# ibrahimhroob/SPS

Measured on AMD Instinct MI355X. Metric: scans/sec @100k pts, 0.1 m voxel, higher is better.
Workload: dtype f32; 1 GPU; BASELINE config 2: single ~100k-pt LiDAR-like scan + variant-B submap, 0.1 m voxel, CustomMinkUNet14 fp32, 1 scan per step per GPU (4 distinct scans cycled); scan_points=100824, rows=153557, streams_per_gpu=8, compact_arenas=True

## Files before the change

### sps_amd/csrc/conv_kernels.inc.h

```cpp

typedef float floatx4 __attribute__((ext_vector_type(4)));

struct ConvArgs {
  const float *in;
  float *out;
  const float *Wu;
  const float *scale;
  const float *shift;
  const float *res;
  const int *nbr;
  const uint32_t *tmask;
  const int *n_out;
  const int *abort_flag;
  int out_rows;
  int64_t ldn;
  int ldi, ldo, ldr;
  int K, cin, cout, NT, upk;
  int relu, S;
  float inv_upk;
  float in_const;
  uint32_t in_bytes, wu_bytes, nbr_bytes;
  int tile_cap;
  int trace_on;
  const float *in2;
// ... 829 lines not shown
#pragma unroll
          for (int i = 0; i < 4; ++i)
            rv[i] = __uint_as_float(__builtin_amdgcn_raw_buffer_load_b32(
                rsR, child[i] >= 0 ? ((uint32_t)child[i] * (uint32_t)a.ldr + (uint32_t)col) * 4u : 0xFFFFFFFFu, 0, 0));
        }
#pragma unroll
        for (int i = 0; i < 4; ++i) {
          if (child[i] < 0) continue;
          float y = acc[nt][i] * esc[nt] + esh[nt];
          y += rv[i];
          if (a.relu) y = fmaxf(y, 0.f);
          a.out[(size_t)child[i] * a.ldo + col] = y;
        }
      }
    }
  }
}

__global__ __launch_bounds__(256) void k_conv0_fused(const int *__restrict__ n_out, LevelView L,
                                                      const float *__restrict__ W, const float *__restrict__ scale,
                                                      const float *__restrict__ shift, float in_const,
                                                      float *__restrict__ out, int ldo, int relu, TileOrderArgs to, int g0) {
  __shared__ float w_s[128 * 8];
  const int gto = (int)gridDim.x - g0;
  if ((int)blockIdx.x < gto) {
    const int which = (int)blockIdx.x;
    if (which < NLV - TILE_ORDER_FIRST_LEVEL)
      tile_order_body(to, which);
    else
      px_order_body(to, which - (NLV - TILE_ORDER_FIRST_LEVEL));
    return;
  }
  const int bid = (int)blockIdx.x - gto;
  if (n_out[ABORT]) return;
  for (int i = threadIdx.x; i < 128 * 8; i += blockDim.x) w_s[i] = i < 125 * 8 ? W[i] : 0.f;
  __syncthreads();
  const int n = *n_out;
  const int ntiles = (n + 15) >> 4;
  const int lane = threadIdx.x & 63, wave = __builtin_amdgcn_readfirstlane((int)(threadIdx.x >> 6));
  const int r = lane & 15, q = lane >> 4;
  const float esc = r < 8 ? scale[r] : 0.f, esh = r < 8 ? shift[r] : 0.f;
  const __amdgpu_buffer_rsrc_t rsM = __builtin_amdgcn_make_buffer_rsrc((void *)L.bmask, 0, (int)0xFFFFFFFEu, 0x00020000);
  for (int tile = bid * 4 + wave; tile < ntiles; tile += g0 * 4) {
    const int row0 = tile * 16;
    const int u = row0 + r;
    uint32_t bm[4] = {0u, 0u, 0u, 0u};
#if defined(SPS_ABLATE_C0FETCH)
    bm[0] = bm[1] = 0x0F0F0F0Fu;
    if (false) {
      const int blk = L.vblock[u];
#else
    if (u < n) {
      const int blk = L.vblock[u];
#endif
      const int bit = L.vbit[u];
      const int px = bit & 3, py = (bit >> 2) & 3, pz = bit >> 4;
      const int lx = px < 2 ? -1 : 0, ly = py < 2 ? -1 : 0, lz = pz < 2 ? -1 : 0;
      const int ysel = q & 1, zsel = q >> 1;
      const int *adj = L.badj + (size_t)blk * 81 + 27 + (lz + zsel + 1) * 9 + (ly + ysel + 1) * 3 + (lx + 1);
      const int nb0 = adj[0], nb1 = adj[1];
      const u32x2 M0 = __builtin_amdgcn_raw_buffer_load_b64(rsM, nb0 >= 0 ? (uint32_t)nb0 * 8u : 0xFFFFFFFFu, 0, 0);
      const u32x2 M1 = __builtin_amdgcn_raw_buffer_load_b64(rsM, nb1 >= 0 ? (uint32_t)nb1 * 8u : 0xFFFFFFFFu, 0, 0);
      const uint32_t m0lo = M0.x, m0hi = M0.y, m1lo = M1.x, m1hi = M1.y;
      const int ysplit = 4 * (ly + 1), zsplit = 4 * (lz + 1);
      const int ty0 = ysel ? ysplit : py - 2, ty1 = ysel ? py + 2 : ysplit - 1;
      const int tz0 = zsel ? zsplit : pz - 2, tz1 = zsel ? pz + 2 : zsplit - 1;
      const int xs = px - 2 - 4 * lx;
#pragma unroll 1
      for (int iz = 0; iz < 4; ++iz) {
        const int tz = tz0 + iz;
        const bool hiw = (tz & 2) != 0;
        const uint32_t w0 = hiw ? m0hi : m0lo, w1 = hiw ? m1hi : m1lo;
        uint32_t plane = 0u;
#pragma unroll
        for (int iy = 0; iy < 4; ++iy) {
          const int ty = ty0 + iy;
          const bool on = tz <= tz1 && ty <= ty1;
          const int sh = ((tz & 1) << 4) | ((ty & 3) << 2);
          const uint32_t n0 = (w0 >> sh) & 0xFu, n1 = (w1 >> sh) & 0xFu;
          const uint32_t pres = on ? (((n0 | (n1 << 4)) >> xs) & 0x1Fu) : 0u;
          plane |= pres << (5 * iy);
        }
        const int k0 = 5 * ((ty0 - py + 2) + 5 * (tz - pz + 2));
        const unsigned long long wide = (unsigned long long)plane << (k0 & 31);
        const int wi = (k0 >> 5) & 3;
        bm[0] |= wi == 0 ? (uint32_t)wide : 0u;
        bm[1] |= wi == 1 ? (uint32_t)wide : (wi == 0 ? (uint32_t)(wide >> 32) : 0u);
        bm[2] |= wi == 2 ? (uint32_t)wide : (wi == 1 ? (uint32_t)(wide >> 32) : 0u);
// ... 173 lines not shown
```

### sps_amd/csrc/grid_kernels.inc.h

```cpp

typedef unsigned int u32x2 __attribute__((ext_vector_type(2)));
constexpr int SCAN_BLOCK = 1024;

struct BHash {
  uint64_t *keys;
  unsigned long long *mask;
  int *first;
  int *rank;
  uint32_t *occ;
  uint32_t hmask;
  uint32_t hshift;
};

constexpr uint32_t BH_X = 0x9E3779B1u, BH_Y = 0x85EBCA77u, BH_Z = 0xC2B2AE3Du, BH_T = 0x27D4EB2Fu;
__device__ inline uint32_t bhash32(uint64_t key) {
  return (uint32_t)(key & 0x3FFFF) * BH_X + (uint32_t)((key >> 18) & 0x3FFFF) * BH_Y + (uint32_t)((key >> 36) & 0x3FFFF) * BH_Z +
         (uint32_t)(key >> 54) * BH_T;
}

__device__ inline int bhash_insert(const BHash &h, uint64_t key) {
  uint32_t s = bhash32(key) >> h.hshift;
  while (true) {
    unsigned long long prev = atomicCAS(reinterpret_cast<unsigned long long *>(&h.keys[s]),
                                        (unsigned long long)KEY_EMPTY, (unsigned long long)key);
// ... 106 lines not shown
  uint64_t *bkey[NLV];
  unsigned long long *bmask[NLV];
  int *bbase[NLV];
  uint4 *bmb[NLV];
  int *bparent[NLV];
  int *bchild[NLV];
  int *badj[NLV];
  int *vblock[NLV];
  unsigned char *vbit[NLV];
  int *counts;
  unsigned long long *agg;
  int agg_stride;
  uint32_t gen;
  const int *n_dev;
  int capl[NLV], bcapl[NLV];
  int *err;
};

constexpr int ABORT = 15;

__device__ inline int block_reduce_sum(int v, int *lds) {
  const int lane = threadIdx.x & 63, wave = threadIdx.x >> 6;
  for (int o = 32; o > 0; o >>= 1) v += __shfl_down(v, o, 64);
  if (lane == 0) lds[wave] = v;
  __syncthreads();
  int tot = 0;
  const int nw = blockDim.x >> 6;
  for (int i = 0; i < nw; ++i) tot += lds[i];
  __syncthreads();
  return tot;
}

constexpr int TICKET = 16, TOCC = 24, N_COUNTERS = 32;

__device__ inline unsigned long long agg_pack(uint32_t gen, int t0, int t1) {
  return ((unsigned long long)gen << 32) | ((unsigned long long)(uint32_t)t1 << 13) | (unsigned long long)(uint32_t)t0;
}
constexpr int SCAN_SPIN_MAX = 1 << 22;
__device__ inline int2 scan_lookback(const unsigned long long *agg, int id, uint32_t gen, int *lds, int *err) {
  if constexpr (SPS_ABLATE_FE & 2) return make_int2(0, 0);
  int p0 = 0, p1 = 0;
  for (int i = threadIdx.x; i < id; i += SCAN_BLOCK) {
    unsigned long long v = __hip_atomic_load(agg + i, __ATOMIC_RELAXED, __HIP_MEMORY_SCOPE_AGENT);
    for (int spin = 0; (uint32_t)(v >> 32) != gen; ++spin) {
      if (spin == SCAN_SPIN_MAX) {
        atomicOr(err, 16);
        v = 0ull;
        break;
      }
      __builtin_amdgcn_s_sleep(1);
      v = __hip_atomic_load(agg + i, __ATOMIC_RELAXED, __HIP_MEMORY_SCOPE_AGENT);
    }
    p0 += (int)(v & 0x1FFFull);
    p1 += (int)((v >> 13) & 0x7FFFFull);
  }
  const int b0 = block_reduce_sum(p0, lds);
  const int b1 = block_reduce_sum(p1, lds);
  return make_int2(b0, b1);
}
__device__ inline int2 block_exclusive_scan2(int v0, int v1, int2 *wave_off, int2 &tot) {
  const int lane = threadIdx.x & 63, wave = threadIdx.x >> 6;
  int i0 = v0, i1 = v1;
  for (int o = 1; o < 64; o <<= 1) {
    const int t0 = __shfl_up(i0, o, 64), t1 = __shfl_up(i1, o, 64);
    if (lane >= o) {
      i0 += t0;
// ... 152 lines not shown
            for (int i = 0; i < 2; ++i)
              if (m & (0x0000000000330033ull << (2 * i + 8 * jj + 32 * kk)))
                pm |= 1ull << ((2 * oz + kk) * 16 + (2 * oy + jj) * 4 + (2 * ox + i));
      } else {
        const uint32_t px = (bx >> (l - 2)) & 3, py = (by >> (l - 2)) & 3, pz = (bz >> (l - 2)) & 3;
        pm = 1ull << ((pz << 4) | (py << 2) | px);
      }
    }
    const int r = k.wg_rank0 + j;
    int sl = 0;
    if constexpr (!(SPS_ABLATE_FE & 4))
      sl = wave_run_insert(a.h[l], pkey, ok, (uint32_t)pm, (uint32_t)(pm >> 32), r);
    if (ok) a.sslot[l][r] = sl;
  }
#if defined(SPS_FE_TRACE)
  __syncthreads();
  FE_STAMP(0, 6);
#endif
}

constexpr int RANK_ITEMS = 1;
__global__ __launch_bounds__(SCAN_BLOCK) void k_rank_blocks_rows(PyramidArgs a, int gsb, int n0, int *__restrict__ inv) {
  __shared__ int lds[SCAN_BLOCK / 64];
  __shared__ int2 wave_off[SCAN_BLOCK / 64];
  __shared__ int sh_id;
  if ((int)blockIdx.x < 4 * gsb) {
    const int nblk = a.counts[8];
    if (((int)blockIdx.x % gsb) * (SCAN_BLOCK * RANK_ITEMS) >= nblk) return;
    Ranked k;
    rank_pass<RANK_ITEMS>(a, 1 + (int)blockIdx.x / gsb, nblk, k, lds, wave_off, &sh_id);
    FE_STAMP(1, 4);
    return;
  }
  if (a.counts[ABORT]) return;
  FE_STAMP(1, 0);
  const int n = a.n_dev ? min(n0, *a.n_dev) : n0;
  const int p = ((int)blockIdx.x - 4 * gsb) * SCAN_BLOCK + (int)threadIdx.x;
  if (p >= n) return;
  const int s = a.sslot[0][p];
  int row = -1;
  if (s >= 0) {
    const BHash &h = a.h[0];
    const int r = h.rank[s];
    const int bit = a.sbit0[p];
    row = a.bbase[0][r] + __popcll(h.mask[s] & ((1ull << bit) - 1ull));
    a.vblock[0][row] = r;
    a.vbit[0][row] = (unsigned char)bit;
  }
  inv[p] = row;
  FE_STAMP(1, 6);
}

__device__ inline void link_levels(const PyramidArgs &a, int l, int bx, int nbx) {
  const int n = a.counts[8 + l];
  for (int r = bx * 256 + (int)threadIdx.x; r < n; r += nbx * 256) {
    const uint64_t key = a.bkey[l][r];
    const uint32_t bx = (uint32_t)(key & 0x3FFFF), by = (uint32_t)((key >> 18) & 0x3FFFF),
                   bz = (uint32_t)((key >> 36) & 0x3FFFF);
    const uint64_t bt = key & (0x3FFull << 54);
    const uint64_t pkey = bt | ((uint64_t)(bz >> 1) << 36) | ((uint64_t)(by >> 1) << 18) | (uint64_t)(bx >> 1);
    const int ps = bhash_find(a.h[l + 1], pkey);
    const int pr = a.h[l + 1].rank[ps];
    a.bparent[l][r] = pr;
    a.bchild[l + 1][(size_t)pr * 8 + ((bx & 1) | ((by & 1) << 1) | ((bz & 1) << 2))] = r;
    if (l == 0) {
      const unsigned long long m = a.bmask[0][r];
      int sj[NLV], brj[NLV], basej[NLV];
      unsigned long long pmj[NLV];
#pragma unroll
      for (int j = 1; j < NLV; ++j) sj[j] = a.sslot[j][r];
#pragma unroll
      for (int j = 1; j < NLV; ++j) {
        brj[j] = a.h[j].rank[sj[j]];
        pmj[j] = a.h[j].mask[sj[j]];
      }
#pragma unroll
      for (int j = 1; j < NLV; ++j) basej[j] = a.bbase[j][brj[j]];
#pragma unroll
      for (int j = 1; j < NLV; ++j) {
        const int br = brj[j];
        const unsigned long long pmask = pmj[j];
        const int base = basej[j];
        if (j == 1) {
          const uint32_t ox = bx & 1, oy = by & 1, oz = bz & 1;
#pragma unroll
          for (int k = 0; k < 2; ++k)
#pragma unroll
            for (int jj = 0; jj < 2; ++jj)
#pragma unroll
              for (int i = 0; i < 2; ++i)
                if (m & (0x0000000000330033ull << (2 * i + 8 * jj + 32 * k))) {
                  const int bit = (int)((2 * oz + k) * 16 + (2 * oy + jj) * 4 + (2 * ox + i));
                  const int row = base + __popcll(pmask & ((1ull << bit) - 1ull));
                  a.vblock[1][row] = br;
                  a.vbit[1][row] = (unsigned char)bit;
                }
        } else {
          const uint32_t px = (bx >> (j - 2)) & 3, py = (by >> (j - 2)) & 3, pz = (bz >> (j - 2)) & 3;
          const int bit = (int)((pz << 4) | (py << 2) | px);
          const int row = base + __popcll(pmask & ((1ull << bit) - 1ull));
          a.vblock[j][row] = br;
          a.vbit[j][row] = (unsigned char)bit;
        }
      }
    }
  }
}

constexpr int LINK_PER = 3;
#if defined(SPS_FE_TRACE)
__device__ unsigned long long g_link_trace[2 * 16384];
struct LinkStamp {
  __device__ LinkStamp() { if (threadIdx.x == 0 && blockIdx.x < 16384) g_link_trace[2 * blockIdx.x] = wall_clock64(); }
  __device__ ~LinkStamp() { if (threadIdx.x == 0 && blockIdx.x < 16384) g_link_trace[2 * blockIdx.x + 1] = wall_clock64(); }
};
#endif
__global__ __launch_bounds__(256) void k_link_adj(PyramidArgs a, int gb, int c1, int c2, int c3, int c4, int c5) {
  if (a.counts[ABORT]) return;
#if defined(SPS_FE_TRACE)
  LinkStamp stamp;
#endif
  if ((int)blockIdx.x < 4 * gb) {
    link_levels(a, (int)blockIdx.x / gb, (int)blockIdx.x % gb, gb);
    return;
  }
  const int bx = (int)blockIdx.x - 4 * gb;
  const int idx = bx < c1 ? 0 : bx < c2 ? 1 : bx < c3 ? 2 : bx < c4 ? 3 : 4;
  const int level = NLV - 1 - idx;
  const int lo = idx == 0 ? 0 : idx == 1 ? c1 : idx == 2 ? c2 : idx == 3 ? c3 : c4;
  const int hi = idx == 0 ? c1 : idx == 1 ? c2 : idx == 2 ? c3 : idx == 3 ? c4 : c5;
  const int total = a.counts[8 + level] * 27;
  const int lim = 1 << (16 - level);
  const BHash h = a.h[level];
  const uint32_t tocc = reinterpret_cast<const uint32_t *>(a.counts)[TOCC];
  const uint64_t *__restrict__ bkey = a.bkey[level];
  int *__restrict__ badj = a.badj[level];
  const __amdgpu_buffer_rsrc_t rsOcc = __builtin_amdgcn_make_buffer_rsrc((void *)h.occ, 0, (int)0xFFFFFFFEu, 0x00020000);
  const __amdgpu_buffer_rsrc_t rsKeys = __builtin_amdgcn_make_buffer_rsrc((void *)h.keys, 0, (int)0xFFFFFFFEu, 0x00020000);
  const __amdgpu_buffer_rsrc_t rsRank = __builtin_amdgcn_make_buffer_rsrc((void *)h.rank, 0, (int)0xFFFFFFFEu, 0x00020000);
  for (int i = (bx - lo) * 256 + (int)threadIdx.x; i < total; i += (hi - lo) * 256) {
    const int r = i / 27, g = i - r * 27;
    const int dy = g % 3 - 1, dz = (g / 3) % 3 - 1, dt = g / 9 - 1;
    const uint64_t key = bkey[r];
    const int kx = (int)(key & 0x3FFFF), ky = (int)((key >> 18) & 0x3FFFF) + dy, kz = (int)((key >> 36) & 0x3FFFF) + dz,
              tt = (int)((key >> 54) & 0x1F) + dt;
    const bool gok = ky >= 0 && ky < lim && kz >= 0 && kz < lim && tt >= 0 && tt < 32 && ((tocc >> tt) & 1u);
    const uint64_t gkey = key + ((uint64_t)(int64_t)dy << 18) + ((uint64_t)(int64_t)dz << 36) + ((uint64_t)(int64_t)dt << 54);
    const uint32_t ghash = bhash32(key) + (uint32_t)dy * BH_Y + (uint32_t)dz * BH_Z + (uint32_t)dt * BH_T;
    uint64_t nk[LINK_PER];
    uint32_t sl[LINK_PER];
    int res[LINK_PER];
    bool probe[LINK_PER];
#pragma unroll
    for (int j = 0; j < LINK_PER; ++j) {
      const int dx = j - 1;
      const bool self = dx == 0 && g == 13;
      res[j] = self ? r : -1;
      probe[j] = !(SPS_ABLATE_FE & 8) && gok && !self && kx + dx >= 0 && kx + dx < lim;
      nk[j] = gkey + (uint64_t)(int64_t)dx;
      sl[j] = (ghash + (uint32_t)dx * BH_X) >> h.hshift;
    }
    uint32_t ow[LINK_PER];
#pragma unroll
    for (int j = 0; j < LINK_PER; ++j) ow[j] = __builtin_amdgcn_raw_buffer_load_b32(rsOcc, probe[j] ? (sl[j] >> 5) * 4u : 0xFFFFFFFFu, 0, 0);
    uint64_t k1[LINK_PER];
#pragma unroll
    for (int j = 0; j < LINK_PER; ++j) {
      probe[j] = probe[j] && ((ow[j] >> (sl[j] & 31)) & 1u);
      const u32x2 kv = __builtin_amdgcn_raw_buffer_load_b64(rsKeys, probe[j] ? sl[j] * 8u : 0xFFFFFFFFu, 0, 0);
      k1[j] = ((uint64_t)kv.y << 32) | kv.x;
    }
    bool hit[LINK_PER];
    int rk[LINK_PER];
#pragma unroll
    for (int j = 0; j < LINK_PER; ++j) {
      hit[j] = probe[j] && k1[j] == nk[j];
      rk[j] = (int)__builtin_amdgcn_raw_buffer_load_b32(rsRank, hit[j] ? sl[j] * 4u : 0xFFFFFFFFu, 0, 0);
    }
#pragma unroll
    for (int j = 0; j < LINK_PER; ++j) {
      if (hit[j]) {
        res[j] = rk[j];
      } else if (probe[j]) {
        const int s2 = bhash_find_from(h, nk[j], (sl[j] + 1) & h.hmask);
        if (s2 >= 0) res[j] = h.rank[s2];
      }
    }
    int *__restrict__ o = badj + (size_t)r * 81 + g * 3;
    if constexpr (SPS_ABLATE_FE & 16) {
      if (g == 13) o[1] = res[1];
    } else {
#pragma unroll
      for (int j = 0; j < LINK_PER; ++j) o[j] = res[j];
    }
  }
}

__device__ inline void bhash_cleanup(const PyramidArgs &a, int l, int bx, int nbx) {
  const int n = a.counts[8 + l];
  const BHash h = a.h[l];
  if (a.counts[ABORT]) {
    const uint32_t slots = h.hmask + 1u;
    for (uint32_t s = (uint32_t)bx * 256u + threadIdx.x; s < slots; s += (uint32_t)nbx * 256u) {
      h.keys[s] = KEY_EMPTY;
      h.mask[s] = 0ull;
      h.first[s] = 0x7F7F7F7F;
      if ((s & 31u) == 0u) h.occ[s >> 5] = 0u;
    }
    return;
  }
  for (int r = bx * 256 + (int)threadIdx.x; r < n; r += nbx * 256) {
    const int s = a.bslot[l][r];
    h.keys[s] = KEY_EMPTY;
    h.mask[s] = 0ull;
// ... 6 lines not shown
```

### sps_amd/csrc/map_kernels.inc.h

```cpp

enum NbrKind { NBR_3333 = 0, NBR_5551 = 1 };

typedef unsigned int u32x4 __attribute__((ext_vector_type(4)));

struct LevelView {
  const int *vblock;
  const unsigned char *vbit;
  const uint64_t *bkey;
  const unsigned long long *bmask;
  const int *bbase;
  const int *badj;
  const int *bparent;
  const int *bchild;
  const uint4 *bmb;
};

__device__ inline bool tile_mask_or(uint32_t *tmask, int u, int k, bool present) {
  const unsigned long long bal = __ballot(present);
  const int lane = threadIdx.x & 63;
  const bool any = ((bal >> (lane & 48)) & 0xFFFFull) != 0ull;
  if ((lane & 15) == 0 && any) atomicOr(&tmask[(size_t)(u >> 4) * 4 + (k >> 5)], 1u << (k & 31));
  return any;
}

// ... 24 lines not shown
  local = bid - a.chunk_off[l];
  return l;
}

template <int R>
__device__ inline void lookup_run(const LevelView &L, int u, int dy, int dz, int dt, int k0, int *__restrict__ nbr,
                                  int64_t ldn, uint32_t *__restrict__ tmask) {
  const int r = L.vblock[u];
  const int bit = L.vbit[u];
  const int px = bit & 3, ty = ((bit >> 2) & 3) + dy, tz = (bit >> 4) + dz;
  const int ad0 = (dt + 1) * 27 + ((tz >> 2) + 1) * 9 + ((ty >> 2) + 1) * 3 + 1;
  const int nbit0 = ((tz & 3) << 4) | ((ty & 3) << 2);
  int last_bo = 99, base = 0;
  unsigned long long mk = 0ull;
#pragma unroll
  for (int dx = -R; dx <= R; ++dx) {
    const int tx = px + dx;
    const int bo = tx >> 2;
    if (bo != last_bo) {
      last_bo = bo;
      const int nb = L.badj[(size_t)r * 81 + ad0 + bo];
      mk = nb >= 0 ? L.bmask[nb] : 0ull;
      base = nb >= 0 ? L.bbase[nb] : 0;
    }
    const int nbit = nbit0 | (tx & 3);
    int row = -1;
    if ((mk >> nbit) & 1ull) row = base + __popcll(mk & ((1ull << nbit) - 1ull));
    const int k = k0 + dx + R;
    if (tile_mask_or(tmask, u, k, row >= 0)) nbr[(size_t)k * ldn + u] = row;
  }
}

template <bool TM, bool RB>
__device__ inline void build_nbr3_t(const MapsArgs &a, int l, int local, int nchunks, int slice) {
  const int n = a.counts[l];
  const LevelView L = a.L[l];
  int *__restrict__ nbr = a.nbr3[l];
  uint32_t *__restrict__ tmask = a.tm3[l];
  const int64_t ldn = a.ldn[l];
  const int lane = threadIdx.x & 63;
  const int nround = (n + 63) & ~63;
  uint32_t *__restrict__ rbe = a.rb_e[l];
  unsigned char *__restrict__ rbk = a.rb_k[l];
  int *__restrict__ rbc = a.rb_cnt[l];
  const uint32_t tocc = reinterpret_cast<const uint32_t *>(a.counts)[TOCC];
  constexpr uint32_t OOR = 0xFFFFFFFFu;
  const __amdgpu_buffer_rsrc_t rsAdj = __builtin_amdgcn_make_buffer_rsrc((void *)L.badj, 0, (int)0xFFFFFFFEu, 0x00020000);
  const __amdgpu_buffer_rsrc_t rsBmb = __builtin_amdgcn_make_buffer_rsrc((void *)L.bmb, 0, (int)0xFFFFFFFEu, 0x00020000);
  for (int u = local * 256 + (int)threadIdx.x; u < nround; u += nchunks * 256) {
    const bool ok = u < n;
    const int r_raw = L.vblock[u];
    const int bit_raw = L.vbit[u];
    const int r = ok ? r_raw : 0;
    const int bit = ok ? bit_raw : 0;
    const int px = bit & 3, py = (bit >> 2) & 3, pz = bit >> 4;
    const int nt = ok ? (int)((L.bkey[r] >> 54) & 0x1F) + slice - 1 : -1;
    const bool act = nt >= 0 && nt < 32 && ((tocc >> nt) & 1u);
    if (!__any(act)) {
      if (TM && (lane & 15) == 0 && ok) tmask[(size_t)(u >> 4) * 4 + slice] = 0u;
      if (RB && lane == 0) rbc[(size_t)(u >> 6) * 4 + slice] = 0;
      continue;
    }
    const uint32_t adj4 = ((uint32_t)r * 81u + (uint32_t)slice * 27u) * 4u;
    const int sx = px == 0 ? -1 : (px == 3 ? 1 : 0), sy = py == 0 ? -1 : (py == 3 ? 1 : 0), sz = pz == 0 ? -1 : (pz == 3 ? 1 : 0);
    uint32_t mlo[8], mhi[8];
    int bs[8], nbv[8];
#pragma unroll
    for (int c = 0; c < 8; ++c) {
      const bool need = act && (!(c & 1) || sx != 0) && (!(c & 2) || sy != 0) && (!(c & 4) || sz != 0);
      const int e = (((c & 4) ? sz : 0) + 1) * 9 + (((c & 2) ? sy : 0) + 1) * 3 + (((c & 1) ? sx : 0) + 1);
      const int v = (int)__builtin_amdgcn_raw_buffer_load_b32(rsAdj, (need && !(SPS_ABLATE_FE & 32)) ? adj4 + (uint32_t)e * 4u : OOR, 0, 0);
      nbv[c] = need ? v : -1;
    }
#pragma unroll
    for (int c = 0; c < 8; ++c) {
      const u32x4 q = __builtin_amdgcn_raw_buffer_load_b128(rsBmb, (nbv[c] >= 0 && !(SPS_ABLATE_FE & 32)) ? (uint32_t)nbv[c] * 16u : OOR, 0, 0);
      mlo[c] = q.x, mhi[c] = q.y, bs[c] = (int)q.z;
      if constexpr (SPS_ABLATE_FE & 32) mlo[c] = 0x0F0F0F0Fu & (uint32_t)(nbv[c] + 1), mhi[c] = mlo[c];
    }
    bool oxv[3];
    uint32_t txl[3], txm[3];
#pragma unroll
    for (int d = 0; d < 3; ++d) {
      const int tx = px + d - 1;
      oxv[d] = (tx >> 2) != 0;
      txl[d] = (uint32_t)(tx & 3);
      txm[d] = (1u << txl[d]) - 1u;
    }
    uint32_t m = 0u;
    int cb = 0;
    uint32_t kinfo = 0u;
    uint32_t *__restrict__ eb = RB ? rbe + ((size_t)(u >> 6) * PX_CH_MAX + (size_t)slice * PX_SEG_CH) * 16 : nullptr;
    unsigned char *__restrict__ kb = RB ? rbk + (size_t)(u >> 6) * PX_KSTRIDE + slice * 112 : nullptr;
#pragma unroll 1
    for (int dz = -1; dz <= ((SPS_ABLATE_FE & 128) ? -2 : 1); ++dz) {
      const int tz = pz + dz;
      const bool oz = (tz >> 2) != 0;
      const bool half = (tz & 2) != 0;
      uint32_t zlo[4], zhi[4];
      int zb[4];
#pragma unroll
      for (int k = 0; k < 4; ++k) zlo[k] = oz ? mlo[k + 4] : mlo[k], zhi[k] = oz ? mhi[k + 4] : mhi[k], zb[k] = oz ? bs[k + 4] : bs[k];
#pragma unroll
      for (int dy = -1; dy <= 1; ++dy) {
        const int ty = py + dy;
        const bool oy = (ty >> 2) != 0;
        const uint32_t sh = (uint32_t)((((tz & 1) << 4) | ((ty & 3) << 2)));
        uint32_t nib[2];
        int pre[2];
// ... 14 lines not shown
          const int jj = (dx + 1) + 3 * (dy + 1);
          const int j = jj + 9 * (dz + 1);
          const unsigned long long bal = __ballot(present);
          if constexpr (TM) {
            const bool any = ((bal >> (lane & 48)) & 0xFFFFull) != 0ull;
            if (any && ok && nbr && !(SPS_ABLATE_FE & 64)) nbr[(size_t)(27 * slice + j) * ldn + u] = row;
            m |= any ? 1u << j : 0u;
          }
          if constexpr (RB) {
            if (bal != 0ull) {
              const int cnt = __popcll(bal);
              const int below = (int)__builtin_amdgcn_mbcnt_hi((uint32_t)(bal >> 32), __builtin_amdgcn_mbcnt_lo((uint32_t)bal, 0u));
              const int pos = present ? below : cnt + lane - below;
              if ((present || pos < ((cnt + 15) & ~15)) && !(SPS_ABLATE_FE & 64)) eb[cb * 16 + pos] = present ? ((uint32_t)row << 7) | (uint32_t)lane : PX_PAD;
              const int nch = (cnt + 15) >> 4;
              kinfo = lane == j ? (uint32_t)cb | ((uint32_t)nch << 16) : kinfo;
              cb += nch;
            }
          }
        }
      }
    }
    if constexpr (RB) {
      const int first = (int)(kinfo & 0xFFFFu), nch = lane < 27 ? (int)(kinfo >> 16) : 0;
#pragma unroll
      for (int i = 0; i < 4; ++i)
        if (i < nch) kb[first + i] = (unsigned char)(27 * slice + lane);
      if (lane == 0) rbc[(size_t)(u >> 6) * 4 + slice] = (SPS_ABLATE_FE & 64) ? 0 : cb;
    }
    if (TM && (lane & 15) == 0 && ok) tmask[(size_t)(u >> 4) * 4 + slice] = m;
  }
}

__device__ inline void build_nbr3(const MapsArgs &a, int bid, int slice) {
  int local;
  const int l = level_of_chunk(a, 0, local, bid);
  const int nchunks = a.chunk_off[l + 1] - a.chunk_off[l];
  const bool rb = a.rb_e[l] != nullptr, tm = a.nbr3[l] != nullptr || !rb;
  if (rb && tm) build_nbr3_t<true, true>(a, l, local, nchunks, slice);
  else if (rb) build_nbr3_t<false, true>(a, l, local, nchunks, slice);
  else build_nbr3_t<true, false>(a, l, local, nchunks, slice);
}

__device__ inline bool tile_mask_test(const uint32_t *__restrict__ tmask, int u, int k, bool slice_words) {
  const int w = slice_words ? k / 27 : k >> 5, b = slice_words ? k - 27 * w : k & 31;
  return (tmask[(size_t)(u >> 4) * 4 + w] >> b) & 1u;
}

__global__ __launch_bounds__(256) void k_build_nbr5(const int *__restrict__ n_out, LevelView L, int *__restrict__ nbr,
                                                     int64_t ldn, uint32_t *__restrict__ tmask) {
  const int n = *n_out;
  const int c = blockIdx.y;
  const int dy = c % 5 - 2, dz = c / 5 - 2;
  for (int u = blockIdx.x * blockDim.x + threadIdx.x; u < n; u += gridDim.x * blockDim.x)
    lookup_run<2>(L, u, dy, dz, 0, 5 * c, nbr, ldn, tmask);
}

__device__ inline void build_stride_maps(const MapsArgs &a, int bid) {
  int local;
  const int f = level_of_chunk(a, 0, local, bid);
  if (f >= NLV - 1) return;
  const int c = f + 1;
  const int nchunks = a.chunk_off[f + 1] - a.chunk_off[f];
  const LevelView F = a.L[f], C = a.L[c];
  const int nf = a.counts[f], nc = a.counts[c];
  const int lane = threadIdx.x & 63;
  for (int v = local * 256 + (int)threadIdx.x; v < nf; v += nchunks * 256) {
    const int r = F.vblock[v];
    const int bit = F.vbit[v];
    const int px = bit & 3, py = (bit >> 2) & 3, pz = bit >> 4;
    const uint64_t key = F.bkey[r];
    const int ox = (int)(key & 1), oy = (int)((key >> 18) & 1), oz = (int)((key >> 36) & 1);
    const int pr = F.bparent[r];
    const int pbit = ((oz * 2 + (pz >> 1)) << 4) | ((oy * 2 + (py >> 1)) << 2) | (ox * 2 + (px >> 1));
    a.parent_row[c][v] = C.bbase[pr] + __popcll(C.bmask[pr] & ((1ull << pbit) - 1ull));
  }
  const int ncr = (nc + 63) & ~63;
  const __amdgpu_buffer_rsrc_t rsFmb = __builtin_amdgcn_make_buffer_rsrc((void *)F.bmb, 0, (int)0xFFFFFFFEu, 0x00020000);
  for (int u = local * 256 + (int)threadIdx.x; u < ncr; u += nchunks * 256) {
    const bool ok = u < nc;
    int px = 0, py = 0, pz = 0, base = 0;
    unsigned long long mk = 0ull;
    if (ok) {
      const int r = C.vblock[u];
      const int bit = C.vbit[u];
      px = bit & 3, py = (bit >> 2) & 3, pz = bit >> 4;
      const int cb = C.bchild[(size_t)r * 8 + ((px >> 1) | ((py >> 1) << 1) | ((pz >> 1) << 2))];
      const u32x4 mb = __builtin_amdgcn_raw_buffer_load_b128(rsFmb, cb >= 0 ? (uint32_t)cb * 16u : 0xFFFFFFFFu, 0, 0);
      mk = ((unsigned long long)mb.y << 32) | mb.x;
      base = (int)mb.z;
    }
    uint32_t m = 0u;
#pragma unroll
    for (int k = 0; k < 8; ++k) {
      const int dx = k & 1, dy = (k >> 1) & 1, dz = (k >> 2) & 1;
      const int cbit = ((((pz & 1) << 1) + dz) << 4) | ((((py & 1) << 1) + dy) << 2) | (((px & 1) << 1) + dx);
      int row = -1;
      if ((mk >> cbit) & 1ull) row = base + __popcll(mk & ((1ull << cbit) - 1ull));
      if (ok) a.down[c][(size_t)k * a.ldn[c] + u] = row;
      const unsigned long long bal = __ballot(row >= 0);
      m |= ((bal >> (lane & 48)) & 0xFFFFull) != 0ull ? 1u << k : 0u;
    }
    if ((lane & 15) == 0 && ok) *reinterpret_cast<uint4 *>(a.tmdown[c] + (size_t)(u >> 4) * 4) = make_uint4(m, 0u, 0u, 0u);
  }
}

#if defined(SPS_FE_TRACE)
__device__ unsigned long long g_maps_trace[2 * 16384];
#endif
__global__ __launch_bounds__(256) void k_maps(MapsArgs ma, int nchunk, int n_nbr) {
  if (ma.counts[ABORT]) return;
  const int bid = (int)blockIdx.x;
#if defined(SPS_FE_TRACE)
  if (threadIdx.x == 0 && bid < 16384) g_maps_trace[2 * bid] = wall_clock64();
#endif
  if (bid < n_nbr)
    build_nbr3(ma, bid % nchunk, bid / nchunk);
  else
    build_stride_maps(ma, bid - n_nbr);
#if defined(SPS_FE_TRACE)
  __syncthreads();
  if (threadIdx.x == 0 && bid < 16384) g_maps_trace[2 * bid + 1] = wall_clock64();
#endif
}

__global__ void k_count_pairs_rb(const uint32_t *__restrict__ rb_e, const unsigned char *__restrict__ rb_k,
                                 const int *__restrict__ rb_cnt, const int *__restrict__ n_ptr,
                                 unsigned long long *__restrict__ pairs) {
  const int nst = (*n_ptr + 63) >> 6;
  const int64_t total = (int64_t)nst * 3 * PX_SEG_CH;
  for (int64_t i = (int64_t)blockIdx.x * blockDim.x + threadIdx.x; i < total; i += (int64_t)gridDim.x * blockDim.x) {
    const int st = (int)(i / (3 * PX_SEG_CH)), r = (int)(i - (int64_t)st * (3 * PX_SEG_CH));
    const int seg = r / PX_SEG_CH, lc = r - seg * PX_SEG_CH;
    if (lc >= rb_cnt[(size_t)st * 4 + seg]) continue;
    const uint32_t *e = rb_e + ((size_t)st * PX_CH_MAX + (size_t)seg * PX_SEG_CH + lc) * 16;
    int c = 0;
    for (int j = 0; j < 16; ++j) c += e[j] != PX_PAD;
    atomicAdd(&pairs[rb_k[(size_t)st * PX_KSTRIDE + seg * 112 + lc]], (unsigned long long)c);
  }
}

__global__ void k_export_table(const int *__restrict__ nbr, int64_t ldn, int K, int slice_words, const int *__restrict__ n_ptr,
                               const uint32_t *__restrict__ tmask, int *__restrict__ out) {
  const int n = *n_ptr;
  const int k = blockIdx.y;
  for (int u = blockIdx.x * blockDim.x + threadIdx.x; u < n; u += gridDim.x * blockDim.x)
    out[(size_t)k * n + u] = tile_mask_test(tmask, u, k, slice_words != 0) ? nbr[(size_t)k * ldn + u] : -1;
}

__global__ void k_export_rulebook(const uint32_t *__restrict__ rb_e, const unsigned char *__restrict__ rb_k,
                                  const int *__restrict__ rb_cnt, const int *__restrict__ n_ptr, int *__restrict__ out,
                                  unsigned long long *__restrict__ entries) {
// ... 144 lines not shown
```

Measured before the change: 4081 scans/s.

## Prefetch per-row indices and counters before abort checks across front-end kernels

Several front-end kernels now load the counter block once per lane and read it with readlane. Per-row vblock/vbit/bkey loads are issued before the abort check and software-pipelined one iteration ahead, so memory latency overlaps with the counter read and the loop body. The stride-map kernel merges its two row loops into one and reads the parent base from the packed bmb record. Level-0 parent links reuse the already-computed pyramid ranks instead of a hash probe, and adjacency rank loads are issued alongside the key loads. The trade-off is speculative loads past valid bounds, which rely on buffer bounds and clamping, plus higher register pressure.

```diff
diff --git a/sps_amd/csrc/conv_kernels.inc.h b/sps_amd/csrc/conv_kernels.inc.h
--- a/sps_amd/csrc/conv_kernels.inc.h
+++ b/sps_amd/csrc/conv_kernels.inc.h
@@ -885,28 +885,34 @@
     return;
   }
   const int bid = (int)blockIdx.x - gto;
-  if (n_out[ABORT]) return;
-  for (int i = threadIdx.x; i < 128 * 8; i += blockDim.x) w_s[i] = i < 125 * 8 ? W[i] : 0.f;
-  __syncthreads();
-  const int n = *n_out;
-  const int ntiles = (n + 15) >> 4;
   const int lane = threadIdx.x & 63, wave = __builtin_amdgcn_readfirstlane((int)(threadIdx.x >> 6));
   const int r = lane & 15, q = lane >> 4;
+  const Counters cnt = load_counters(n_out);
+  const int tile0 = bid * 4 + wave;
+  int blk_next = L.vblock[tile0 * 16 + r];
+  int bit_next = L.vbit[tile0 * 16 + r];
+  for (int i = threadIdx.x; i < 128 * 8; i += blockDim.x) w_s[i] = i < 125 * 8 ? W[i] : 0.f;
+  if (cnt[ABORT]) return;
+  __syncthreads();
+  const int n = cnt[0];
+  const int ntiles = (n + 15) >> 4;
   const float esc = r < 8 ? scale[r] : 0.f, esh = r < 8 ? shift[r] : 0.f;
   const __amdgpu_buffer_rsrc_t rsM = __builtin_amdgcn_make_buffer_rsrc((void *)L.bmask, 0, (int)0xFFFFFFFEu, 0x00020000);
-  for (int tile = bid * 4 + wave; tile < ntiles; tile += g0 * 4) {
+  for (int tile = tile0; tile < ntiles; tile += g0 * 4) {
     const int row0 = tile * 16;
     const int u = row0 + r;
+    const int blk_cur = blk_next, bit_cur = bit_next;
+    if (tile + g0 * 4 < ntiles) blk_next = L.vblock[u + g0 * 64], bit_next = L.vbit[u + g0 * 64];
     uint32_t bm[4] = {0u, 0u, 0u, 0u};
 #if defined(SPS_ABLATE_C0FETCH)
     bm[0] = bm[1] = 0x0F0F0F0Fu;
     if (false) {
-      const int blk = L.vblock[u];
+      const int blk = blk_cur;
 #else
     if (u < n) {
-      const int blk = L.vblock[u];
-#endif
-      const int bit = L.vbit[u];
+      const int blk = blk_cur;
+#endif
+      const int bit = bit_cur;
       const int px = bit & 3, py = (bit >> 2) & 3, pz = bit >> 4;
       const int lx = px < 2 ? -1 : 0, ly = py < 2 ? -1 : 0, lz = pz < 2 ? -1 : 0;
       const int ysel = q & 1, zsel = q >> 1;
diff --git a/sps_amd/csrc/grid_kernels.inc.h b/sps_amd/csrc/grid_kernels.inc.h
--- a/sps_amd/csrc/grid_kernels.inc.h
+++ b/sps_amd/csrc/grid_kernels.inc.h
@@ -162,6 +162,15 @@
 }
 
 constexpr int TICKET = 16, TOCC = 24, N_COUNTERS = 32;
+struct Counters {
+  int v;
+  __device__ int operator[](int i) const { return __builtin_amdgcn_readlane(v, i); }
+};
+__device__ inline Counters load_counters(const int *counts) {
+  Counters c;
+  c.v = counts[threadIdx.x & (N_COUNTERS - 1)];
+  return c;
+}
 
 __device__ inline unsigned long long agg_pack(uint32_t gen, int t0, int t1) {
   return ((unsigned long long)gen << 32) | ((unsigned long long)(uint32_t)t1 << 13) | (unsigned long long)(uint32_t)t0;
@@ -380,17 +389,18 @@
     FE_STAMP(1, 4);
     return;
   }
-  if (a.counts[ABORT]) return;
+  const int p = ((int)blockIdx.x - 4 * gsb) * SCAN_BLOCK + (int)threadIdx.x;
+  const int s = a.sslot[0][p];
+  const int bit = a.sbit0[p];
+  const Counters cnt = load_counters(a.counts);
+  if (cnt[ABORT]) return;
   FE_STAMP(1, 0);
   const int n = a.n_dev ? min(n0, *a.n_dev) : n0;
-  const int p = ((int)blockIdx.x - 4 * gsb) * SCAN_BLOCK + (int)threadIdx.x;
   if (p >= n) return;
-  const int s = a.sslot[0][p];
   int row = -1;
   if (s >= 0) {
     const BHash &h = a.h[0];
     const int r = h.rank[s];
-    const int bit = a.sbit0[p];
     row = a.bbase[0][r] + __popcll(h.mask[s] & ((1ull << bit) - 1ull));
     a.vblock[0][row] = r;
     a.vbit[0][row] = (unsigned char)bit;
@@ -399,18 +409,26 @@
   FE_STAMP(1, 6);
 }
 
-__device__ inline void link_levels(const PyramidArgs &a, int l, int bx, int nbx) {
-  const int n = a.counts[8 + l];
+__device__ inline void link_levels(const PyramidArgs &a, int l, int n, int bx, int nbx) {
   for (int r = bx * 256 + (int)threadIdx.x; r < n; r += nbx * 256) {
     const uint64_t key = a.bkey[l][r];
     const uint32_t bx = (uint32_t)(key & 0x3FFFF), by = (uint32_t)((key >> 18) & 0x3FFFF),
                    bz = (uint32_t)((key >> 36) & 0x3FFFF);
-    const uint64_t bt = key & (0x3FFull << 54);
-    const uint64_t pkey = bt | ((uint64_t)(bz >> 1) << 36) | ((uint64_t)(by >> 1) << 18) | (uint64_t)(bx >> 1);
-    const int ps = bhash_find(a.h[l + 1], pkey);
-    const int pr = a.h[l + 1].rank[ps];
-    a.bparent[l][r] = pr;
-    a.bchild[l + 1][(size_t)pr * 8 + ((bx & 1) | ((by & 1) << 1) | ((bz & 1) << 2))] = r;
+    const int oct = (int)((bx & 1) | ((by & 1) << 1) | ((bz & 1) << 2));
+    if (l != 0 || (SPS_ABLATE_FE & 4)) {
+      const uint64_t bt = key & (0x3FFull << 54);
+      const uint64_t pkey = bt | ((uint64_t)(bz >> 1) << 36) | ((uint64_t)(by >> 1) << 18) | (uint64_t)(bx >> 1);
+      const BHash &h = a.h[l + 1];
+      const uint32_t s = bhash32(pkey) >> h.hshift;
+      const uint64_t k1 = h.keys[s];
+      int pr = h.rank[s];
+      if (k1 != pkey) {
+        const int ps = bhash_find_from(h, pkey, (s + 1) & h.hmask);
+        pr = ps >= 0 ? h.rank[ps] : 0;
+      }
+      a.bparent[l][r] = pr;
+      a.bchild[l + 1][(size_t)pr * 8 + oct] = r;
+    }
     if (l == 0) {
       const unsigned long long m = a.bmask[0][r];
       int sj[NLV], brj[NLV], basej[NLV];
@@ -424,6 +442,10 @@
       }
 #pragma unroll
       for (int j = 1; j < NLV; ++j) basej[j] = a.bbase[j][brj[j]];
+      if constexpr (!(SPS_ABLATE_FE & 4)) {
+        a.bparent[0][r] = brj[1];
+        a.bchild[1][(size_t)brj[1] * 8 + oct] = r;
+      }
 #pragma unroll
       for (int j = 1; j < NLV; ++j) {
         const int br = brj[j];
@@ -464,32 +486,40 @@
 };
 #endif
 __global__ __launch_bounds__(256) void k_link_adj(PyramidArgs a, int gb, int c1, int c2, int c3, int c4, int c5) {
-  if (a.counts[ABORT]) return;
+  const bool links = (int)blockIdx.x < 4 * gb;
+  const int bx = (int)blockIdx.x - 4 * gb;
+  const int idx = bx < c1 ? 0 : bx < c2 ? 1 : bx < c3 ? 2 : bx < c4 ? 3 : 4;
+  const int level = links ? (int)blockIdx.x / gb : NLV - 1 - idx;
+  const Counters cnt = load_counters(a.counts);
+  const int lo = idx == 0 ? 0 : idx == 1 ? c1 : idx == 2 ? c2 : idx == 3 ? c3 : c4;
+  const int hi = idx == 0 ? c1 : idx == 1 ? c2 : idx == 2 ? c3 : idx == 3 ? c4 : c5;
+  const __amdgpu_buffer_rsrc_t rsBkey = __builtin_amdgcn_make_buffer_rsrc((void *)a.bkey[level], 0, a.bcapl[level] * 8, 0x00020000);
+  const int i0 = (bx - lo) * 256 + (int)threadIdx.x;
+  u32x2 kv0 = {0u, 0u};
+  if (!links) kv0 = __builtin_amdgcn_raw_buffer_load_b64(rsBkey, (uint32_t)(i0 / 27) * 8u, 0, 0);
+  if (cnt[ABORT]) return;
+  const int nblocks = cnt[8 + level];
+  const uint32_t tocc = (uint32_t)cnt[TOCC];
 #if defined(SPS_FE_TRACE)
   LinkStamp stamp;
 #endif
-  if ((int)blockIdx.x < 4 * gb) {
-    link_levels(a, (int)blockIdx.x / gb, (int)blockIdx.x % gb, gb);
+  if (links) {
+    link_levels(a, level, nblocks, (int)blockIdx.x % gb, gb);
     return;
   }
-  const int bx = (int)blockIdx.x - 4 * gb;
-  const int idx = bx < c1 ? 0 : bx < c2 ? 1 : bx < c3 ? 2 : bx < c4 ? 3 : 4;
-  const int level = NLV - 1 - idx;
-  const int lo = idx == 0 ? 0 : idx == 1 ? c1 : idx == 2 ? c2 : idx == 3 ? c3 : c4;
-  const int hi = idx == 0 ? c1 : idx == 1 ? c2 : idx == 2 ? c3 : idx == 3 ? c4 : c5;
-  const int total = a.counts[8 + level] * 27;
+  const int total = nblocks * 27;
   const int lim = 1 << (16 - level);
   const BHash h = a.h[level];
-  const uint32_t tocc = reinterpret_cast<const uint32_t *>(a.counts)[TOCC];
-  const uint64_t *__restrict__ bkey = a.bkey[level];
   int *__restrict__ badj = a.badj[level];
   const __amdgpu_buffer_rsrc_t rsOcc = __builtin_amdgcn_make_buffer_rsrc((void *)h.occ, 0, (int)0xFFFFFFFEu, 0x00020000);
   const __amdgpu_buffer_rsrc_t rsKeys = __builtin_amdgcn_make_buffer_rsrc((void *)h.keys, 0, (int)0xFFFFFFFEu, 0x00020000);
   const __amdgpu_buffer_rsrc_t rsRank = __builtin_amdgcn_make_buffer_rsrc((void *)h.rank, 0, (int)0xFFFFFFFEu, 0x00020000);
-  for (int i = (bx - lo) * 256 + (int)threadIdx.x; i < total; i += (hi - lo) * 256) {
+  const int step = (hi - lo) * 256;
+  for (int i = i0; i < total; i += step) {
     const int r = i / 27, g = i - r * 27;
     const int dy = g % 3 - 1, dz = (g / 3) % 3 - 1, dt = g / 9 - 1;
-    const uint64_t key = bkey[r];
+    const uint64_t key = ((uint64_t)kv0.y << 32) | kv0.x;
+    kv0 = __builtin_amdgcn_raw_buffer_load_b64(rsBkey, (uint32_t)((i + step) / 27) * 8u, 0, 0);
     const int kx = (int)(key & 0x3FFFF), ky = (int)((key >> 18) & 0x3FFFF) + dy, kz = (int)((key >> 36) & 0x3FFFF) + dz,
               tt = (int)((key >> 54) & 0x1F) + dt;
     const bool gok = ky >= 0 && ky < lim && kz >= 0 && kz < lim && tt >= 0 && tt < 32 && ((tocc >> tt) & 1u);
@@ -512,22 +542,17 @@
 #pragma unroll
     for (int j = 0; j < LINK_PER; ++j) ow[j] = __builtin_amdgcn_raw_buffer_load_b32(rsOcc, probe[j] ? (sl[j] >> 5) * 4u : 0xFFFFFFFFu, 0, 0);
     uint64_t k1[LINK_PER];
+    int rk[LINK_PER];
 #pragma unroll
     for (int j = 0; j < LINK_PER; ++j) {
       probe[j] = probe[j] && ((ow[j] >> (sl[j] & 31)) & 1u);
       const u32x2 kv = __builtin_amdgcn_raw_buffer_load_b64(rsKeys, probe[j] ? sl[j] * 8u : 0xFFFFFFFFu, 0, 0);
       k1[j] = ((uint64_t)kv.y << 32) | kv.x;
-    }
-    bool hit[LINK_PER];
-    int rk[LINK_PER];
+      rk[j] = (int)__builtin_amdgcn_raw_buffer_load_b32(rsRank, probe[j] ? sl[j] * 4u : 0xFFFFFFFFu, 0, 0);
+    }
 #pragma unroll
     for (int j = 0; j < LINK_PER; ++j) {
-      hit[j] = probe[j] && k1[j] == nk[j];
-      rk[j] = (int)__builtin_amdgcn_raw_buffer_load_b32(rsRank, hit[j] ? sl[j] * 4u : 0xFFFFFFFFu, 0, 0);
-    }
-#pragma unroll
-    for (int j = 0; j < LINK_PER; ++j) {
-      if (hit[j]) {
+      if (probe[j] && k1[j] == nk[j]) {
         res[j] = rk[j];
       } else if (probe[j]) {
         const int s2 = bhash_find_from(h, nk[j], (sl[j] + 1) & h.hmask);
diff --git a/sps_amd/csrc/map_kernels.inc.h b/sps_amd/csrc/map_kernels.inc.h
--- a/sps_amd/csrc/map_kernels.inc.h
+++ b/sps_amd/csrc/map_kernels.inc.h
@@ -80,8 +80,8 @@
 }
 
 template <bool TM, bool RB>
-__device__ inline void build_nbr3_t(const MapsArgs &a, int l, int local, int nchunks, int slice) {
-  const int n = a.counts[l];
+__device__ inline void build_nbr3_t(const MapsArgs &a, int l, int local, int nchunks, int slice, int n, uint32_t tocc,
+                                    __amdgpu_buffer_rsrc_t rsVb, __amdgpu_buffer_rsrc_t rsVt, int r_raw, int bit_raw) {
   const LevelView L = a.L[l];
   int *__restrict__ nbr = a.nbr3[l];
   uint32_t *__restrict__ tmask = a.tm3[l];
@@ -91,38 +91,39 @@
   uint32_t *__restrict__ rbe = a.rb_e[l];
   unsigned char *__restrict__ rbk = a.rb_k[l];
   int *__restrict__ rbc = a.rb_cnt[l];
-  const uint32_t tocc = reinterpret_cast<const uint32_t *>(a.counts)[TOCC];
   constexpr uint32_t OOR = 0xFFFFFFFFu;
   const __amdgpu_buffer_rsrc_t rsAdj = __builtin_amdgcn_make_buffer_rsrc((void *)L.badj, 0, (int)0xFFFFFFFEu, 0x00020000);
   const __amdgpu_buffer_rsrc_t rsBmb = __builtin_amdgcn_make_buffer_rsrc((void *)L.bmb, 0, (int)0xFFFFFFFEu, 0x00020000);
-  for (int u = local * 256 + (int)threadIdx.x; u < nround; u += nchunks * 256) {
+  const uint32_t *__restrict__ bkey_hi = reinterpret_cast<const uint32_t *>(L.bkey) + 1;
+  const int u0 = local * 256 + (int)threadIdx.x, ustep = nchunks * 256;
+  for (int u = u0; u < nround; u += ustep, r_raw = (int)__builtin_amdgcn_raw_buffer_load_b32(rsVb, (uint32_t)u * 4u, 0, 0),
+           bit_raw = (int)__builtin_amdgcn_raw_buffer_load_b8(rsVt, (uint32_t)u, 0, 0)) {
     const bool ok = u < n;
-    const int r_raw = L.vblock[u];
-    const int bit_raw = L.vbit[u];
     const int r = ok ? r_raw : 0;
     const int bit = ok ? bit_raw : 0;
     const int px = bit & 3, py = (bit >> 2) & 3, pz = bit >> 4;
-    const int nt = ok ? (int)((L.bkey[r] >> 54) & 0x1F) + slice - 1 : -1;
+    const uint32_t adj4 = ((uint32_t)r * 81u + (uint32_t)slice * 27u) * 4u;
+    const uint32_t khi = bkey_hi[2 * (size_t)r];
+    const int sx = px == 0 ? -1 : (px == 3 ? 1 : 0), sy = py == 0 ? -1 : (py == 3 ? 1 : 0), sz = pz == 0 ? -1 : (pz == 3 ? 1 : 0);
+    uint32_t mlo[8], mhi[8];
+    int bs[8], nbv[8];
+#pragma unroll
+    for (int c = 0; c < 8; ++c) {
+      const bool need = ok && (!(c & 1) || sx != 0) && (!(c & 2) || sy != 0) && (!(c & 4) || sz != 0);
+      const int e = (((c & 4) ? sz : 0) + 1) * 9 + (((c & 2) ? sy : 0) + 1) * 3 + (((c & 1) ? sx : 0) + 1);
+      const int v = (int)__builtin_amdgcn_raw_buffer_load_b32(rsAdj, (need && !(SPS_ABLATE_FE & 32)) ? adj4 + (uint32_t)e * 4u : OOR, 0, 0);
+      nbv[c] = need ? v : -1;
+    }
+    const int nt = ok ? (int)((khi >> 22) & 0x1F) + slice - 1 : -1;
     const bool act = nt >= 0 && nt < 32 && ((tocc >> nt) & 1u);
     if (!__any(act)) {
       if (TM && (lane & 15) == 0 && ok) tmask[(size_t)(u >> 4) * 4 + slice] = 0u;
       if (RB && lane == 0) rbc[(size_t)(u >> 6) * 4 + slice] = 0;
       continue;
     }
-    const uint32_t adj4 = ((uint32_t)r * 81u + (uint32_t)slice * 27u) * 4u;
-    const int sx = px == 0 ? -1 : (px == 3 ? 1 : 0), sy = py == 0 ? -1 : (py == 3 ? 1 : 0), sz = pz == 0 ? -1 : (pz == 3 ? 1 : 0);
-    uint32_t mlo[8], mhi[8];
-    int bs[8], nbv[8];
 #pragma unroll
     for (int c = 0; c < 8; ++c) {
-      const bool need = act && (!(c & 1) || sx != 0) && (!(c & 2) || sy != 0) && (!(c & 4) || sz != 0);
-      const int e = (((c & 4) ? sz : 0) + 1) * 9 + (((c & 2) ? sy : 0) + 1) * 3 + (((c & 1) ? sx : 0) + 1);
-      const int v = (int)__builtin_amdgcn_raw_buffer_load_b32(rsAdj, (need && !(SPS_ABLATE_FE & 32)) ? adj4 + (uint32_t)e * 4u : OOR, 0, 0);
-      nbv[c] = need ? v : -1;
-    }
-#pragma unroll
-    for (int c = 0; c < 8; ++c) {
-      const u32x4 q = __builtin_amdgcn_raw_buffer_load_b128(rsBmb, (nbv[c] >= 0 && !(SPS_ABLATE_FE & 32)) ? (uint32_t)nbv[c] * 16u : OOR, 0, 0);
+      const u32x4 q = __builtin_amdgcn_raw_buffer_load_b128(rsBmb, (act && nbv[c] >= 0 && !(SPS_ABLATE_FE & 32)) ? (uint32_t)nbv[c] * 16u : OOR, 0, 0);
       mlo[c] = q.x, mhi[c] = q.y, bs[c] = (int)q.z;
       if constexpr (SPS_ABLATE_FE & 32) mlo[c] = 0x0F0F0F0Fu & (uint32_t)(nbv[c] + 1), mhi[c] = mlo[c];
     }
@@ -203,14 +204,22 @@
   }
 }
 
-__device__ inline void build_nbr3(const MapsArgs &a, int bid, int slice) {
+__device__ inline void build_nbr3(const MapsArgs &a, int bid, int slice, const Counters cnt) {
   int local;
   const int l = level_of_chunk(a, 0, local, bid);
   const int nchunks = a.chunk_off[l + 1] - a.chunk_off[l];
   const bool rb = a.rb_e[l] != nullptr, tm = a.nbr3[l] != nullptr || !rb;
-  if (rb && tm) build_nbr3_t<true, true>(a, l, local, nchunks, slice);
-  else if (rb) build_nbr3_t<false, true>(a, l, local, nchunks, slice);
-  else build_nbr3_t<true, false>(a, l, local, nchunks, slice);
+  const __amdgpu_buffer_rsrc_t rsVb = __builtin_amdgcn_make_buffer_rsrc((void *)a.L[l].vblock, 0, (int)a.ldn[l] * 4, 0x00020000);
+  const __amdgpu_buffer_rsrc_t rsVt = __builtin_amdgcn_make_buffer_rsrc((void *)a.L[l].vbit, 0, (int)a.ldn[l], 0x00020000);
+  const int u0 = local * 256 + (int)threadIdx.x;
+  const int r0 = (int)__builtin_amdgcn_raw_buffer_load_b32(rsVb, (uint32_t)u0 * 4u, 0, 0);
+  const int bit0 = (int)__builtin_amdgcn_raw_buffer_load_b8(rsVt, (uint32_t)u0, 0, 0);
+  if (cnt[ABORT]) return;
+  const int n = cnt[l];
+  const uint32_t tocc = (uint32_t)cnt[TOCC];
+  if (rb && tm) build_nbr3_t<true, true>(a, l, local, nchunks, slice, n, tocc, rsVb, rsVt, r0, bit0);
+  else if (rb) build_nbr3_t<false, true>(a, l, local, nchunks, slice, n, tocc, rsVb, rsVt, r0, bit0);
+  else build_nbr3_t<true, false>(a, l, local, nchunks, slice, n, tocc, rsVb, rsVt, r0, bit0);
 }
 
 __device__ inline bool tile_mask_test(const uint32_t *__restrict__ tmask, int u, int k, bool slice_words) {
@@ -227,40 +236,51 @@
     lookup_run<2>(L, u, dy, dz, 0, 5 * c, nbr, ldn, tmask);
 }
 
-__device__ inline void build_stride_maps(const MapsArgs &a, int bid) {
+__device__ inline void build_stride_maps(const MapsArgs &a, int bid, const Counters cnt) {
   int local;
   const int f = level_of_chunk(a, 0, local, bid);
   if (f >= NLV - 1) return;
   const int c = f + 1;
   const int nchunks = a.chunk_off[f + 1] - a.chunk_off[f];
   const LevelView F = a.L[f], C = a.L[c];
-  const int nf = a.counts[f], nc = a.counts[c];
   const int lane = threadIdx.x & 63;
-  for (int v = local * 256 + (int)threadIdx.x; v < nf; v += nchunks * 256) {
-    const int r = F.vblock[v];
-    const int bit = F.vbit[v];
-    const int px = bit & 3, py = (bit >> 2) & 3, pz = bit >> 4;
-    const uint64_t key = F.bkey[r];
-    const int ox = (int)(key & 1), oy = (int)((key >> 18) & 1), oz = (int)((key >> 36) & 1);
-    const int pr = F.bparent[r];
-    const int pbit = ((oz * 2 + (pz >> 1)) << 4) | ((oy * 2 + (py >> 1)) << 2) | (ox * 2 + (px >> 1));
-    a.parent_row[c][v] = C.bbase[pr] + __popcll(C.bmask[pr] & ((1ull << pbit) - 1ull));
-  }
-  const int ncr = (nc + 63) & ~63;
+  const __amdgpu_buffer_rsrc_t rsFvb = __builtin_amdgcn_make_buffer_rsrc((void *)F.vblock, 0, (int)a.ldn[f] * 4, 0x00020000);
+  const __amdgpu_buffer_rsrc_t rsFvt = __builtin_amdgcn_make_buffer_rsrc((void *)F.vbit, 0, (int)a.ldn[f], 0x00020000);
+  const __amdgpu_buffer_rsrc_t rsCvb = __builtin_amdgcn_make_buffer_rsrc((void *)C.vblock, 0, (int)a.ldn[c] * 4, 0x00020000);
+  const __amdgpu_buffer_rsrc_t rsCvt = __builtin_amdgcn_make_buffer_rsrc((void *)C.vbit, 0, (int)a.ldn[c], 0x00020000);
   const __amdgpu_buffer_rsrc_t rsFmb = __builtin_amdgcn_make_buffer_rsrc((void *)F.bmb, 0, (int)0xFFFFFFFEu, 0x00020000);
-  for (int u = local * 256 + (int)threadIdx.x; u < ncr; u += nchunks * 256) {
-    const bool ok = u < nc;
-    int px = 0, py = 0, pz = 0, base = 0;
-    unsigned long long mk = 0ull;
-    if (ok) {
-      const int r = C.vblock[u];
-      const int bit = C.vbit[u];
-      px = bit & 3, py = (bit >> 2) & 3, pz = bit >> 4;
-      const int cb = C.bchild[(size_t)r * 8 + ((px >> 1) | ((py >> 1) << 1) | ((pz >> 1) << 2))];
-      const u32x4 mb = __builtin_amdgcn_raw_buffer_load_b128(rsFmb, cb >= 0 ? (uint32_t)cb * 16u : 0xFFFFFFFFu, 0, 0);
-      mk = ((unsigned long long)mb.y << 32) | mb.x;
-      base = (int)mb.z;
-    }
+  const __amdgpu_buffer_rsrc_t rsCmb = __builtin_amdgcn_make_buffer_rsrc((void *)C.bmb, 0, (int)0xFFFFFFFEu, 0x00020000);
+  const int i0 = local * 256 + (int)threadIdx.x, istep = nchunks * 256;
+  int fr_raw = (int)__builtin_amdgcn_raw_buffer_load_b32(rsFvb, (uint32_t)i0 * 4u, 0, 0);
+  int fbit_raw = (int)__builtin_amdgcn_raw_buffer_load_b8(rsFvt, (uint32_t)i0, 0, 0);
+  int cr_raw = (int)__builtin_amdgcn_raw_buffer_load_b32(rsCvb, (uint32_t)i0 * 4u, 0, 0);
+  int cbit_raw = (int)__builtin_amdgcn_raw_buffer_load_b8(rsCvt, (uint32_t)i0, 0, 0);
+  if (cnt[ABORT]) return;
+  const int nf = cnt[f], nc = cnt[c];
+  const int nboth = (max(nf, nc) + 63) & ~63;
+  for (int u = i0; u < nboth; u += istep) {
+    const bool okf = u < nf, ok = u < nc;
+    const int fr = okf ? fr_raw : 0, fbit = okf ? fbit_raw : 0;
+    const int cr = ok ? cr_raw : 0, cbit0 = ok ? cbit_raw : 0;
+    const int px = cbit0 & 3, py = (cbit0 >> 2) & 3, pz = cbit0 >> 4;
+    const uint64_t fkey = F.bkey[fr];
+    const int pr_raw = F.bparent[fr];
+    const int cb_raw = C.bchild[(size_t)cr * 8 + ((px >> 1) | ((py >> 1) << 1) | ((pz >> 1) << 2))];
+    fr_raw = (int)__builtin_amdgcn_raw_buffer_load_b32(rsFvb, (uint32_t)(u + istep) * 4u, 0, 0);
+    fbit_raw = (int)__builtin_amdgcn_raw_buffer_load_b8(rsFvt, (uint32_t)(u + istep), 0, 0);
+    cr_raw = (int)__builtin_amdgcn_raw_buffer_load_b32(rsCvb, (uint32_t)(u + istep) * 4u, 0, 0);
+    cbit_raw = (int)__builtin_amdgcn_raw_buffer_load_b8(rsCvt, (uint32_t)(u + istep), 0, 0);
+    const u32x4 pmb = __builtin_amdgcn_raw_buffer_load_b128(rsCmb, okf ? (uint32_t)pr_raw * 16u : 0xFFFFFFFFu, 0, 0);
+    const u32x4 mb = __builtin_amdgcn_raw_buffer_load_b128(rsFmb, (ok && cb_raw >= 0) ? (uint32_t)cb_raw * 16u : 0xFFFFFFFFu, 0, 0);
+    if (okf) {
+      const int fx = fbit & 3, fy = (fbit >> 2) & 3, fz = fbit >> 4;
+      const int ox = (int)(fkey & 1), oy = (int)((fkey >> 18) & 1), oz = (int)((fkey >> 36) & 1);
+      const int pbit = ((oz * 2 + (fz >> 1)) << 4) | ((oy * 2 + (fy >> 1)) << 2) | (ox * 2 + (fx >> 1));
+      const unsigned long long pm = ((unsigned long long)pmb.y << 32) | pmb.x;
+      a.parent_row[c][u] = (int)pmb.z + __popcll(pm & ((1ull << pbit) - 1ull));
+    }
+    const unsigned long long mk = ((unsigned long long)mb.y << 32) | mb.x;
+    const int base = (int)mb.z;
     uint32_t m = 0u;
 #pragma unroll
     for (int k = 0; k < 8; ++k) {
@@ -280,15 +300,15 @@
 __device__ unsigned long long g_maps_trace[2 * 16384];
 #endif
 __global__ __launch_bounds__(256) void k_maps(MapsArgs ma, int nchunk, int n_nbr) {
-  if (ma.counts[ABORT]) return;
+  const Counters cnt = load_counters(ma.counts);
   const int bid = (int)blockIdx.x;
 #if defined(SPS_FE_TRACE)
   if (threadIdx.x == 0 && bid < 16384) g_maps_trace[2 * bid] = wall_clock64();
 #endif
   if (bid < n_nbr)
-    build_nbr3(ma, bid % nchunk, bid / nchunk);
+    build_nbr3(ma, bid % nchunk, bid / nchunk, cnt);
   else
-    build_stride_maps(ma, bid - n_nbr);
+    build_stride_maps(ma, bid - n_nbr, cnt);
 #if defined(SPS_FE_TRACE)
   __syncthreads();
   if (threadIdx.x == 0 && bid < 16384) g_maps_trace[2 * bid + 1] = wall_clock64();
```

Result: slower. 4010 scans/s (-1.7%).
